# finsberg/fenicsx-beat

Measured on AMD Instinct MI355X. Metric: node_updates_per_sec, higher is better.
Workload: dtype f64

## Files before the change

fenicsx-beat_amd/csrc/beat_pde_rr.hip:

```cpp
#include "beat_pde_internal.h"

#include <algorithm>
#include <cmath>
#include <cstddef>
#include <cstdlib>

namespace {
using namespace beat_pde_detail;

constexpr int SEG = 62;

struct Coef {
  double c[15];
};

struct RGeom {
  int nx, ny, nz;
  int64_t plane;
  int ry;
  int nsegx, nrb, nchunks, zc;
  int total_waves, total_blocks;
  int z_lo_phys, z_hi_phys;
  int z_lo, z_hi;
  int part_off;
  int ghost_lo_tz, ghost_hi_tz;
  int nrg;
};

enum { RR_PDOT = 0, RR_RUPD = 1, RR_RHS = 2, RR_UDOT = 3, RR_PRUPD = 4 };

struct RArgs {
  const double* x;
  const double* x2;
  double* y;
  double* y2;
  const double* tab;
  const double* tab2;
  const double* dinv;
  Coef ci, ci2;
  double dinv_i;
  double cm, omt_dt, dt;
  const double* w[BEAT_MAX_STIM];
  double amp[BEAT_MAX_STIM];
  int nstim;
  double* partials;
  double* st;
  double* alphas;
  int slot;
  const double* e;
  const double* taba;
  Coef cia;
};

struct RKernArgs {
  RGeom g;
  RArgs a;
  const double* X;
  const double* X2;
  double* Y;
  double* Y2;
};

__device__ __forceinline__ double from_left(double v) {
  const int lo = __builtin_amdgcn_update_dpp(0, __double2loint(v), 0x138, 0xf, 0xf, true);
  const int hi = __builtin_amdgcn_update_dpp(0, __double2hiint(v), 0x138, 0xf, 0xf, true);
  return __hiloint2double(hi, lo);
}
__device__ __forceinline__ double from_right(double v) {
  const int lo = __builtin_amdgcn_update_dpp(0, __double2loint(v), 0x130, 0xf, 0xf, true);
  const int hi = __builtin_amdgcn_update_dpp(0, __double2hiint(v), 0x130, 0xf, 0xf, true);
  return __hiloint2double(hi, lo);
}

#ifndef BEAT_RR_BUF
#define BEAT_RR_BUF 2
#endif
typedef int rr_v2i __attribute__((ext_vector_type(2)));
[[maybe_unused]] constexpr unsigned RR_OOB = 0x80000000u;
#ifndef BEAT_RR_NT
#define BEAT_RR_NT 2
#endif
__device__ __forceinline__ void rr_store(double* p, double v) {
#if BEAT_RR_NT & 2
  __builtin_nontemporal_store(v, p);
#else
  *p = v;
#endif
}
__device__ __forceinline__ double rr_buf_load(const double* base, unsigned bytes, unsigned off) {
  const __amdgpu_buffer_rsrc_t r = __builtin_amdgcn_make_buffer_rsrc((void*)base, 0, (int)bytes, 0x00020000);
  const rr_v2i v = __builtin_amdgcn_raw_buffer_load_b64(r, (int)off, 0, (BEAT_RR_NT & 1) ? 2 : 0);
  return __hiloint2double(v.y, v.x);
}

#ifndef BEAT_RR_ALIGN
#define BEAT_RR_ALIGN 1
#endif
__device__ __forceinline__ double from_left_h(double v, double h, int src_lane) {
  const int lo = __builtin_amdgcn_update_dpp(__builtin_amdgcn_readlane(__double2loint(h), src_lane), __double2loint(v), 0x138, 0xf, 0xf, false);
  const int hi = __builtin_amdgcn_update_dpp(__builtin_amdgcn_readlane(__double2hiint(h), src_lane), __double2hiint(v), 0x138, 0xf, 0xf, false);
  return __hiloint2double(hi, lo);
}
__device__ __forceinline__ double from_right_h(double v, double h, int src_lane) {
  const int lo = __builtin_amdgcn_update_dpp(__builtin_amdgcn_readlane(__double2loint(h), src_lane), __double2loint(v), 0x130, 0xf, 0xf, false);
  const int hi = __builtin_amdgcn_update_dpp(__builtin_amdgcn_readlane(__double2hiint(h), src_lane), __double2hiint(v), 0x130, 0xf, 0xf, false);
  return __hiloint2double(hi, lo);
}
#ifndef BEAT_RR_ALIGN_RHS
#define BEAT_RR_ALIGN_RHS 0
#endif
constexpr bool rr_aligned_mode(int mode) {
  return BEAT_RR_ALIGN == 1 && BEAT_RR_BUF != 0 && (mode == 0 || mode == 1 || mode == 3 || mode == 4 || (mode == 2 && BEAT_RR_ALIGN_RHS == 1));
}

__device__ __forceinline__ int axis_type3(int i, int n, int lo_phys, int hi_phys) {
  if (n == 1 && lo_phys && hi_phys) return 1;
  if (i == 0 && lo_phys) return 0;
  if (i == n - 1 && hi_phys) return 2;
  return 1;
}

__device__ __forceinline__ int xcd_block(int b, int total) {
  const int per = (total + 7) >> 3;
  return (b & 7) * per + (b >> 3);
}

#ifndef BEAT_RR_WAVES_RHS
#define BEAT_RR_WAVES_RHS 3
#endif
#ifndef BEAT_RR_WAVES_IT
#define BEAT_RR_WAVES_IT 1
#endif
template <int MODE, int RY, int PD, bool GUESS = false, bool PRED = false>
__global__ __launch_bounds__(BEAT_BLOCK, (GUESS && RY == 2 && PD == 1) ? BEAT_RR_WAVES_RHS : ((MODE == RR_PDOT || MODE == RR_RUPD) && PD == 1 ? BEAT_RR_WAVES_IT : 1)) void rr_kernel(RGeom g, RArgs a, const double* __restrict__ X,
                                                        const double* __restrict__ X2, double* __restrict__ Y,
                                                        double* __restrict__ Y2) {
  constexpr int NR = RY + 2;
  constexpr int NE = GUESS ? NR : 1;
  constexpr bool FORM = MODE == RR_PDOT || MODE == RR_UDOT || MODE == RR_PRUPD;
  constexpr bool OLD = MODE == RR_PDOT || MODE == RR_PRUPD;
  constexpr bool RAW = MODE == RR_UDOT || MODE == RR_PRUPD;
  constexpr int NW = RAW ? RY : 1;
  constexpr bool BUF = BEAT_RR_BUF == 1 || (BEAT_RR_BUF == 2 && (MODE != RR_RHS || BEAT_RR_ALIGN_RHS == 1));
  constexpr bool ALIGNED = rr_aligned_mode(MODE);
  static_assert(!ALIGNED || BUF, "aligned segments come with the raw-buffer loads");
  constexpr int SEGW = ALIGNED ? 64 : SEG;
  static_assert(!GUESS || MODE == RR_RHS, "the initial guess enters the right-hand side only");
  static_assert(!PRED || MODE == RR_PDOT, "the predicted-stop sums come with PDOT only");
  __shared__ double red[4];
  __shared__ double s_dinv[32];
  __shared__ double s_tab[27 * TABW];
  __shared__ double s_tab2[MODE == RR_RHS ? 27 * TABW : 1];
  __shared__ double s_taba[GUESS ? 27 * TABW : 1];
  __shared__ double s_rc[PRED ? 4 * 2 * RY * 64 : 1];
  __shared__ double s_acc[PRED ? 4 * 2 * 64 : 1];
  if (MODE != RR_RHS) {
    if (a.st[STOP] != 0.0) return;
  }
  if (PRED) s_acc[(threadIdx.x >> 6) * 128 + (threadIdx.x & 63)] = s_acc[(threadIdx.x >> 6) * 128 + 64 + (threadIdx.x & 63)] = 0.0;
  for (int i = threadIdx.x; i < 27 * TABW; i += BEAT_BLOCK) {
    s_tab[i] = a.tab[i];
    if (MODE == RR_RHS) s_tab2[i] = a.tab2[i];
    if (GUESS) s_taba[i] = a.taba[i];
  }
  if (threadIdx.x < 27) s_dinv[threadIdx.x] = a.dinv[threadIdx.x];
  __syncthreads();
  const int lane = threadIdx.x & 63;
  const int blk = xcd_block(blockIdx.x, g.total_blocks);
  const int w = blk * 4 + (threadIdx.x >> 6);
  int seg = w % g.nsegx;
  int rb = (w / g.nsegx) % g.nrb;
  int chunk = w / (g.nsegx * g.nrb);
  bool wave_ok = blk < g.total_blocks && w < g.total_waves;
  if (g.nrg > 0) {
    seg = blk % g.nsegx;
    rb = ((blk / g.nsegx) % g.nrg) * 4 + (int)(threadIdx.x >> 6);
    chunk = blk / (g.nsegx * g.nrg);
    wave_ok = blk < g.total_blocks && rb < g.nrb;
  }
  const int gx = seg * SEGW + (ALIGNED ? 0 : -1) + lane;
  const int y0 = rb * RY - 1;
  const int zb = g.z_lo + chunk * g.zc;
  const int ze = wave_ok ? min(zb + g.zc, g.z_hi) : zb;
  const bool x_in = wave_ok && gx >= 0 && gx < g.nx;
  const bool x_out = x_in && (ALIGNED || (lane >= 1 && lane <= SEG));
  const int tx = axis_type3(gx, g.nx, 1, 1);
  bool row_in[NR];
  int txy[NR];
  int off[NR];
  const int cx = min(max(gx, 0), g.nx - 1);
#pragma unroll
  for (int r = 0; r < NR; ++r) {
    const int gy = y0 + r;
    row_in[r] = x_in && gy >= 0 && gy < g.ny;
    txy[r] = tx + 3 * axis_type3(gy, g.ny, 1, 1);
    off[r] = min(max(gy, 0), g.ny - 1) * g.nx + cx;
    if constexpr (BUF) off[r] = row_in[r] ? (int)((unsigned)(gy * g.nx + gx) * 8u) : (int)RR_OOB;
  }
  [[maybe_unused]] const unsigned pbytes = (unsigned)(g.plane * 8);
  [[maybe_unused]] unsigned hoff = RR_OOB;
  [[maybe_unused]] int htxy = 13 % 9;
  if constexpr (ALIGNED) {
    const int hr = lane < 8 ? lane : lane - 8;
    const int hx = lane < 8 ? seg * SEGW - 1 : seg * SEGW + SEGW;
    const int hy = y0 + hr;
    const bool hv = wave_ok && (lane < NR || (lane >= 8 && lane < 8 + NR)) && hx >= 0 && hx < g.nx && hy >= 0 && hy < g.ny;
    hoff = hv ? (unsigned)(hy * g.nx + hx) * 8u : RR_OOB;
    htxy = axis_type3(min(max(hx, 0), g.nx - 1), g.nx, 1, 1) + 3 * axis_type3(min(max(hy, 0), g.ny - 1), g.ny, 1, 1);
  }
  double beta = 0.0, alpha = 0.0;
  if (OLD) beta = a.st[BETA];
  if (MODE == RR_PRUPD) alpha = a.st[ALPHA];
  if (MODE == RR_RUPD) {
    alpha = a.st[RZ] / a.st[PQ];
    if (blockIdx.x == 0 && threadIdx.x == 0) a.alphas[a.slot] = alpha;
  }
  const bool have_old = beta != 0.0;

  double acc0 = 0.0, acc1 = 0.0, acc2 = 0.0;
  double Cm[NR], C0[NR], Cp[NR], ra[PD][NR], rb2[PD][NR];
  double rvn[PD][RY];
  [[maybe_unused]] double Hm = 0.0, H0 = 0.0, Hp = 0.0, rha[PD], rhb[PD];
  [[maybe_unused]] double HEm = 0.0, HE0 = 0.0, HEp = 0.0;
#pragma unroll
  for (int u = 0; u < PD; ++u) rha[u] = rhb[u] = 0.0;
  double Rw0[NW], Rwp[NW];
#pragma unroll
  for (int j = 0; j < NW; ++j) Rw0[j] = Rwp[j] = 0.0;
  double Em[NE], E0[NE], Ep[NE], re1[PD][NE];
#pragma unroll
  for (int r = 0; r < NE; ++r) {
    Em[r] = E0[r] = Ep[r] = 0.0;
#pragma unroll
    for (int u = 0; u < PD; ++u) re1[u][r] = 0.0;
  }
#pragma unroll
  for (int r = 0; r < NR; ++r) {
    Cm[r] = C0[r] = Cp[r] = 0.0;
#pragma unroll
    for (int u = 0; u < PD; ++u) ra[u][r] = rb2[u][r] = 0.0;
  }
#pragma unroll
  for (int u = 0; u < PD; ++u)
#pragma unroll
    for (int j = 0; j < RY; ++j) rvn[u][j] = 0.0;
  for (int zz = zb - 2 - PD; zz < ze; zz += PD) {
#pragma unroll
  for (int u = 0; u < PD; ++u) {
    const int z = zz + u;
    if (z < ze) {
    const int k = z + 1;
    if (k >= zb - 1 && k <= ze) {
      [[maybe_unused]] const bool zok = (k >= 0 || !g.z_lo_phys) && (k < g.nz || !g.z_hi_phys);
      const int tz9 = 9 * (k < 0 ? g.ghost_lo_tz : k >= g.nz ? g.ghost_hi_tz : axis_type3(k, g.nz, g.z_lo_phys, g.z_hi_phys));
      const bool own_plane = (k >= zb && k < ze) || (k == -1 && zb == 0 && !g.z_lo_phys) ||
                             (k == g.nz && ze == g.nz && !g.z_hi_phys);
#pragma unroll
      for (int r = 0; r < NR; ++r) {
        double c = ra[u][r];
        if (RAW && r >= 1 && r <= RY) Rwp[RAW ? r - 1 : 0] = c;
        if (FORM) {
          const int type = txy[r] + tz9;
          const double di = s_dinv[type];
          c = have_old ? fma(beta, rb2[u][r], di * ra[u][r]) : di * ra[u][r];
        }
        if constexpr (!BUF) c = (zok && row_in[r]) ? c : 0.0;
        Cp[r] = c;
        if (GUESS) {
          constexpr int q = GUESS ? 1 : 0;
          if constexpr (BUF)
            Ep[r * q] = c + re1[u][r * q];
          else
            Ep[r * q] = (zok && row_in[r]) ? c + re1[u][r * q] : 0.0;
        }
        if (OLD) {
          if (own_plane && r >= 1 && r <= RY && x_out && row_in[r])
            rr_store(&Y[(int64_t)k * g.plane + (int64_t)(y0 + r) * g.nx + gx], c);
        }
        if (PRED && r >= 1 && r <= RY) s_rc[((((threadIdx.x >> 6) * 2 + (k & 1)) * RY) + r - 1) * 64 + lane] = ra[u][r];
      }
      if constexpr (ALIGNED) {
        double hc = rha[u];
        if (FORM) {
          const double di = s_dinv[htxy + tz9];
          hc = have_old ? fma(beta, rhb[u], di * rha[u]) : di * rha[u];
        }
        Hp = hc;
        if (GUESS) HEp = hc + rhb[u];
      }
    }
    double rv[RY];
    if (MODE == RR_RUPD) {
#pragma unroll
      for (int j = 0; j < RY; ++j) rv[j] = rvn[u][j];
      if (z + PD >= zb && z + PD < ze) {
        const double* __restrict__ br = X2 + (int64_t)(z + PD) * g.plane;
#pragma unroll
        for (int j = 0; j < RY; ++j) rvn[u][j] = BUF ? rr_buf_load(br, pbytes, (unsigned)off[j + 1]) : br[off[j + 1]];
      }
    }
    {
      const int kf = k + PD;
      if (kf >= zb - 1 && kf <= ze) {
        const int cz = min(max(kf, -1), g.nz);
        const double* __restrict__ bx = X + (int64_t)cz * g.plane;
        const double* __restrict__ bx2 = (OLD && have_old) ? X2 + (int64_t)cz * g.plane : bx;
        if constexpr (BUF) {
          const unsigned pb = ((kf >= 0 || !g.z_lo_phys) && (kf < g.nz || !g.z_hi_phys)) ? pbytes : 0u;
#pragma unroll
          for (int r = 0; r < NR; ++r) {
            ra[u][r] = rr_buf_load(bx, pb, (unsigned)off[r]);
            if (OLD) rb2[u][r] = rr_buf_load(bx2, pb, (unsigned)off[r]);
          }
          if constexpr (ALIGNED) {
            rha[u] = rr_buf_load(bx, pb, hoff);
            if (OLD) rhb[u] = rr_buf_load(bx2, pb, hoff);
            if (GUESS) rhb[u] = rr_buf_load(X2 + (int64_t)cz * g.plane, pb, hoff);
          }
          if (GUESS) {
            const double* __restrict__ b1 = X2 + (int64_t)cz * g.plane;
#pragma unroll
            for (int r = 0; r < NR; ++r) re1[u][r < NE ? r : 0] = rr_buf_load(b1, pb, (unsigned)off[r]);
          }
        } else {
#pragma unroll
          for (int r = 0; r < NR; ++r) {
            ra[u][r] = bx[off[r]];
            if (OLD) rb2[u][r] = bx2[off[r]];
          }
          if (GUESS) {
            const double* __restrict__ b1 = X2 + (int64_t)cz * g.plane;
#pragma unroll
            for (int r = 0; r < NR; ++r) re1[u][r < NE ? r : 0] = b1[off[r]];
          }
        }
      }
    }
    if (z >= zb) {
    typedef const __attribute__((address_space(4))) char* KArgPtr;
    KArgPtr ka = (KArgPtr)__builtin_amdgcn_kernarg_segment_ptr();
    asm volatile("" : "+s"(ka));
    const RArgs& az = MODE == RR_RHS ? *(const RArgs*)(ka + offsetof(RKernArgs, a)) : a;
    double L0[NR], R0[NR], Rp[NR], Lm[NR];
#pragma unroll
    for (int r = 0; r < NR - 1; ++r) {
      L0[r] = ALIGNED ? from_left_h(C0[r], H0, r) : from_left(C0[r]);
      Lm[r] = ALIGNED ? from_left_h(Cm[r], Hm, r) : from_left(Cm[r]);
    }
#pragma unroll
    for (int r = 1; r < NR; ++r) {
      R0[r] = ALIGNED ? from_right_h(C0[r], H0, 8 + r) : from_right(C0[r]);
      Rp[r] = ALIGNED ? from_right_h(Cp[r], Hp, 8 + r) : from_right(Cp[r]);
    }
    double eL0[NE], eR0[NE], eRp[NE], eLm[NE];
    if (GUESS) {
#pragma unroll
      for (int r = 0; r < NE - 1; ++r) {
        eL0[r] = ALIGNED ? from_left_h(E0[r], HE0, r) : from_left(E0[r]);
        eLm[r] = ALIGNED ? from_left_h(Em[r], HEm, r) : from_left(Em[r]);
      }
#pragma unroll
      for (int r = 1; r < NE; ++r) {
        eR0[r] = ALIGNED ? from_right_h(E0[r], HE0, 8 + r) : from_right(E0[r]);
        eRp[r] = ALIGNED ? from_right_h(Ep[r], HEp, 8 + r) : from_right(Ep[r]);
      }
    }
    const int tz = axis_type3(z, g.nz, g.z_lo_phys, g.z_hi_phys);
#pragma unroll
    for (int j = 0; j < RY; ++j) {
      const int r = j + 1;
      double v[15];
      v[0] = C0[r];
      v[1] = R0[r];
      v[2] = L0[r];
      v[3] = C0[r + 1];
      v[4] = C0[r - 1];
      v[5] = Cp[r];
      v[6] = Cm[r];
      v[7] = R0[r + 1];
      v[8] = L0[r - 1];
      v[9] = Cp[r + 1];
      v[10] = Cm[r - 1];
      v[11] = Rp[r];
      v[12] = Lm[r];
      v[13] = Rp[r + 1];
      v[14] = Lm[r - 1];
      if (x_out && row_in[r]) {
        const int type = txy[r] + 9 * tz;
        const int64_t gi = (int64_t)z * g.plane + (int64_t)(y0 + r) * g.nx + gx;
        double s = 0.0;
#pragma unroll
        for (int k = 0; k < 15; ++k) s = fma(az.ci.c[k], v[k], s);
        if (MODE == RR_RHS) {
          double s2 = 0.0;
          if (!GUESS) {
#pragma unroll
            for (int k = 0; k < 15; ++k) s2 = fma(az.ci2.c[k], v[k], s2);
          }
          double di = s_dinv[13];
          if (type != 13) {
            s = 0.0;
            s2 = 0.0;
#pragma unroll
            for (int k = 0; k < 15; ++k) {
              s = fma(s_tab[type * TABW + k], v[k], s);
              if (!GUESS) s2 = fma(s_tab2[type * TABW + k], v[k], s2);
            }
            di = s_dinv[type];
          }
          double stim = 0.0;
          for (int k = 0; k < az.nstim; ++k) stim = fma(az.amp[k], az.w[k][gi], stim);
          const double b = GUESS ? fma(az.dt, stim, s) : az.cm * s - az.omt_dt * s2 + az.dt * stim;
          double rr = GUESS ? b : az.dt * (stim - s2);
          if (GUESS) {
            constexpr int q = GUESS ? 1 : 0;
            const int re_ = r * q, rp = (r + 1) * q, rm = (r - 1) * q;
            double ev[15];
            ev[0] = E0[re_];
            ev[1] = eR0[re_];
            ev[2] = eL0[re_];
            ev[3] = E0[rp];
            ev[4] = E0[rm];
            ev[5] = Ep[re_];
            ev[6] = Em[re_];
            ev[7] = eR0[rp];
            ev[8] = eL0[rm];
            ev[9] = Ep[rp];
            ev[10] = Em[rm];
            ev[11] = eRp[re_];
            ev[12] = eLm[re_];
            ev[13] = eRp[rp];
            ev[14] = eLm[rm];
            double se = 0.0;
            if (type != 13) {
#pragma unroll
              for (int k = 0; k < 15; ++k) se = fma(s_taba[type * TABW + k], ev[k], se);
            } else {
#pragma unroll
              for (int k = 0; k < 15; ++k) se = fma(az.cia.c[k], ev[k], se);
            }
            rr -= se;
          }
          const double zz = di * rr;
          rr_store(&Y[gi], rr);
          if (Y2 != nullptr) Y2[gi] = v[0];
          acc0 = fma(b, b, acc0);
          acc1 = fma(rr, zz, acc1);
          acc2 = fma(rr, rr, acc2);
        } else {
          double di = s_dinv[13];
          if (type != 13) {
            s = 0.0;
#pragma unroll
            for (int k = 0; k < 15; ++k) s = fma(s_tab[type * TABW + k], v[k], s);
            di = s_dinv[type];
          }
          if (MODE == RR_PDOT) {
            acc0 = fma(v[0], s, acc0);
            if (PRED) {
              double* sa = &s_acc[(threadIdx.x >> 6) * 128 + lane];
              sa[0] = fma(s_rc[((((threadIdx.x >> 6) * 2 + (z & 1)) * RY) + j) * 64 + lane], s, sa[0]);
              sa[64] = fma(s, s, sa[64]);
            }
          } else if (MODE == RR_UDOT) {
            const double ri = Rw0[RAW ? j : 0];
            acc0 = fma(v[0], s, acc0);
            acc1 = fma(ri, v[0], acc1);
            acc2 = fma(ri, ri, acc2);
          } else if (MODE == RR_PRUPD) {
            rr_store(&Y2[gi], fma(-alpha, s, Rw0[RAW ? j : 0]));
          } else {
            const double ri = fma(-alpha, s, rv[j]);
            rr_store(&Y[gi], ri);
            acc0 = fma(ri * di, ri, acc0);
            acc1 = fma(ri, ri, acc1);
          }
        }
      }
    }
    }
#pragma unroll
    for (int r = 0; r < NR; ++r) {
      Cm[r] = C0[r];
      C0[r] = Cp[r];
    }
    if constexpr (ALIGNED) {
      Hm = H0;
      H0 = Hp;
      if (GUESS) {
        HEm = HE0;
        HE0 = HEp;
      }
    }
    if (GUESS) {
#pragma unroll
      for (int r = 0; r < NE; ++r) {
        Em[r] = E0[r];
        E0[r] = Ep[r];
      }
    }
    if (RAW) {
#pragma unroll
      for (int j = 0; j < NW; ++j) Rw0[j] = Rwp[j];
    }
    }
  }
  }

  if (PRED) {
    acc1 = s_acc[(threadIdx.x >> 6) * 128 + (threadIdx.x & 63)];
    acc2 = s_acc[(threadIdx.x >> 6) * 128 + 64 + (threadIdx.x & 63)];
  }
  if (MODE == RR_PDOT && !PRED) {
    const double s0 = beat_block_sum(acc0, red);
    if (threadIdx.x == 0) a.partials[g.part_off + blockIdx.x] = s0;
  } else if (MODE == RR_RUPD) {
    const double s0 = beat_block_sum(acc0, red);
    const double s1 = beat_block_sum(acc1, red);
    if (threadIdx.x == 0) {
      a.partials[g.part_off + blockIdx.x] = s0;
      a.partials[BEAT_MAX_PARTIALS + g.part_off + blockIdx.x] = s1;
    }
  } else if (MODE == RR_PRUPD) {
  } else {
    const double s0 = beat_block_sum(acc0, red);
    const double s1 = beat_block_sum(acc1, red);
    const double s2 = beat_block_sum(acc2, red);
    if (threadIdx.x == 0) {
      a.partials[g.part_off + blockIdx.x] = s0;
      a.partials[BEAT_MAX_PARTIALS + g.part_off + blockIdx.x] = s1;
      a.partials[2 * BEAT_MAX_PARTIALS + g.part_off + blockIdx.x] = s2;
    }
  }
}

__global__ void rr_next_kernel(double* st) {
  if (st[STOP] != 0.0) return;
  st[BETA] = st[RZN] / st[RZ];
  st[RZ] = st[RZN];
  st[RR] = st[RRN];
  st[ITERS] += 1.0;
  const double tr = st[RTOL] * st[RTOL] * st[BB];
  if (st[RR] <= st[TOL2]) {
    st[STOP] = 1.0;
    st[REASON] = st[RR] <= tr ? 2.0 : 3.0;
  } else if (st[ITERS] >= st[MAXIT]) {
    st[STOP] = 1.0;
    st[REASON] = -3.0;
  }
}

__global__ void rr_merged_next_kernel(double* st, double* alphas, int slot) {
  if (st[STOP] != 0.0) return;
  const double g = st[RZN], d = st[PQ], rr = st[RRN];
  st[RR] = rr;
  const double tr = st[RTOL] * st[RTOL] * st[BB];
  if (rr <= st[TOL2]) {
    st[STOP] = 1.0;
    st[REASON] = rr <= tr ? 2.0 : 3.0;
    return;
  }
  if (st[ITERS] >= st[MAXIT]) {
    st[STOP] = 1.0;
    st[REASON] = -3.0;
    return;
  }
  const bool first = st[ITERS] == 0.0;
  const double beta = first ? 0.0 : g / st[RZ];
  const double alpha = first ? g / d : g / (d - beta * g / st[ALPHA]);
  st[BETA] = beta;
  st[ALPHA] = alpha;
  st[RZ] = g;
  alphas[slot] = alpha;
  st[NUPD] += 1.0;
  st[ITERS] += 1.0;
}

int rr_rows(int64_t nodes) {
  static const int forced = [] {
    const char* e = std::getenv("BEAT_RR_RY");
    const int v = e ? std::atoi(e) : 0;
    return (v == 2 || v == 4) ? v : 0;
  }();
  if (forced) return forced;
  return nodes >= ((int64_t)64 << 20) ? 4 : 2;
}

int rr_target_blocks(int64_t nodes) {
  if (const char* e = std::getenv("BEAT_RR_BLOCKS")) return std::max(1, std::atoi(e));
  return nodes >= ((int64_t)64 << 20) ? 4096 : 2048;
}

int rr_prefetch() {
  static const int pd = [] {
    const char* e = std::getenv("BEAT_RR_PD");
    const int v = e ? std::atoi(e) : 1;
    return (v >= 1 && v <= 3) ? v : 1;
  }();
  return pd;
}

int rr_by_rows_mask() {
  static const int mask = [] {
    const char* e = std::getenv("BEAT_RR_BY_ROWS");
    return e ? std::atoi(e) : 0;
  }();
  return mask;
}

RGeom make_geom(const beat_pde* pde, int z_lo, int z_hi, int part_off, int rows = 0, int mode = -1) {
  const Geom& f = pde->g;
  RGeom g{};
  const int64_t nodes = (int64_t)f.nx * f.ny * f.nz;
  const int RY = g.ry = rows ? rows : rr_rows(nodes);
  g.nx = f.nx;
  g.ny = f.ny;
  g.nz = f.nz;
  g.plane = f.plane;
  g.z_lo_phys = f.z_lo_phys;
  g.z_hi_phys = f.z_hi_phys;
  g.z_lo = z_lo;
  g.z_hi = z_hi;
  g.part_off = part_off;
  g.ghost_lo_tz = pde->ghost_lo_tz;
  g.ghost_hi_tz = pde->ghost_hi_tz;
  const int segw = (mode >= 0 && rr_aligned_mode(mode)) ? 64 : SEG;
  g.nsegx = (f.nx + segw - 1) / segw;
  g.nrb = (f.ny + RY - 1) / RY;
  const int nzr = std::max(0, z_hi - z_lo);
  g.nrg = (mode >= 0 && ((rr_by_rows_mask() >> mode) & 1)) ? (g.nrb + 3) / 4 : 0;
  const int64_t per_layer = g.nrg > 0 ? (int64_t)g.nsegx * g.nrg : ((int64_t)g.nsegx * g.nrb + 3) / 4;
  const int target = rr_target_blocks(nodes);
  int nchunks = (int)std::max<int64_t>(1, (target + per_layer - 1) / per_layer);
  nchunks = std::max(1, std::min(nchunks, nzr));
  g.zc = std::max(1, (nzr + nchunks - 1) / nchunks);
  g.nchunks = (nzr + g.zc - 1) / g.zc;
  while ((int64_t)g.nsegx * g.nrb * g.nchunks > (int64_t)2 * BEAT_MAX_PARTIALS && g.nchunks > 1) {
    g.zc *= 2;
    g.nchunks = (nzr + g.zc - 1) / g.zc;
  }
  g.total_waves = g.nsegx * g.nrb * g.nchunks;
  g.total_blocks = (g.total_waves + 3) / 4;
  if (g.nrg > 0) {
    g.total_blocks = g.nsegx * g.nrg * g.nchunks;
    g.total_waves = g.total_blocks * 4;
  }
  return g;
}

RGeom make_geom(const beat_pde* pde) { return make_geom(pde, 0, pde->g.nz, 0); }

inline int grid_blocks(const RGeom& g) { return ((g.total_blocks + 7) / 8) * 8; }
inline int blocks_written(const RGeom& g) { return g.total_blocks > 0 ? grid_blocks(g) : 0; }

Coef interior_row(const double* tab) {
  Coef c;
  for (int k = 0; k < 15; ++k) c.c[k] = tab[13 * 15 + k];
  return c;
}

RArgs rr_operator_args(const beat_pde* pde, double* dev_st) {
  RArgs a{};
  a.tab = pde->d_tab(0);
  a.dinv = pde->d_dinv();
  a.ci = interior_row(pde->h_A);
  a.dinv_i = pde->h_dinv[13];
  a.partials = pde->ctx->d_partials;
  a.st = dev_st;
  return a;
}

template <int MODE, bool GUESS = false, bool PRED = false>
void launch_rr(const beat_pde* pde, const RGeom& g, const RArgs& a) {
  if (g.total_blocks <= 0) return;
  const dim3 grid((unsigned)grid_blocks(g)), block(BEAT_BLOCK);
  hipStream_t s = pde->ctx->stream;
#define BEAT_RR_LAUNCH(RYV, PDV) \
  BEAT_KERNEL((rr_kernel<MODE, RYV, PDV, GUESS, PRED>), grid, block, 0, s, g, a, a.x, GUESS ? a.e : a.x2, a.y, a.y2)
  const int pd = rr_prefetch();
  if (g.ry == 2) {
    if (pd == 2) BEAT_RR_LAUNCH(2, 2); else if (pd == 3) BEAT_RR_LAUNCH(2, 3); else BEAT_RR_LAUNCH(2, 1);
  } else {
    if (pd == 2) BEAT_RR_LAUNCH(4, 2); else if (pd == 3) BEAT_RR_LAUNCH(4, 3); else BEAT_RR_LAUNCH(4, 1);
  }
#undef BEAT_RR_LAUNCH
}
}

bool beat_rr_available(const beat_pde* pde) {
  if (pde->var || pde->pc_ncoef != 1) return false;
  if (const char* e = std::getenv("BEAT_RR")) {
    if (e[0] == '0') return false;
  }
  const RGeom g = make_geom(pde);
  const RGeom gb = make_geom(pde, 0, 1, 0);
  return (int64_t)grid_blocks(g) + 2 * grid_blocks(gb) <= BEAT_MAX_PARTIALS;
}

int beat_rr_rhs(beat_pde* pde, const double* dev_v_prev, const double* const* host_dev_stim_w, const double* host_stim_amp,
                int n_stim, double* dev_x, double* dev_r, double* dev_st, int part, const PcgStart* start) {
  BEAT_REQUIRE(start == nullptr || part < 0, "only a right-hand side in one part starts the solve");
  const GuessTerms& gt = pde->guess;
  const bool guess = gt.d != nullptr && gt.use_e;
  static const int guess_rows = [] {
    const char* e = std::getenv("BEAT_RR_GUESS_RY");
    const int v = e ? std::atoi(e) : 2;
    return v == 4 ? 4 : 2;
  }();
  const int rows = guess ? guess_rows : 0;
  RArgs a{};
  a.x = dev_v_prev;
  a.y = dev_r;
  a.y2 = (dev_x == dev_v_prev) ? nullptr : dev_x;
  a.tab = pde->d_tab(2);
  a.tab2 = pde->d_tab(3);
  a.dinv = pde->d_dinv();
  a.ci = interior_row(pde->h_mass);
  a.ci2 = interior_row(pde->h_stiff);
  a.dinv_i = pde->h_dinv[13];
  a.cm = pde->C_m;
  a.omt_dt = (1.0 - pde->theta) * pde->dt;
  a.dt = pde->dt;
  beat_fill_stimuli(a, host_dev_stim_w, host_stim_amp, n_stim);
  a.partials = pde->ctx->d_partials;
  a.st = dev_st;
  if (guess) {
    a.tab = pde->d_tab(1);
    a.ci = interior_row(pde->h_B);
    a.e = gt.e;
    a.taba = pde->d_tab(0);
    a.cia = interior_row(pde->h_A);
  }
  auto launch = [&](int z_lo, int z_hi, int part_off) {
    const RGeom g = make_geom(pde, z_lo, z_hi, part_off, rows, RR_RHS);
    if (guess)
      launch_rr<RR_RHS, true>(pde, g, a);
    else
      launch_rr<RR_RHS>(pde, g, a);
    return blocks_written(g);
  };
  int count = 0;
  if (int rc = beat_launch_parts(pde, PASS_RR_RHS, part, launch, &count)) return rc;
  return part == 0 ? BEAT_OK : beat_pde_launch_reduce(pde, count, 3, dev_st, nullptr, ScalarStep::begin(dev_st, start));
}

double beat_rr_predict_bound(const beat_pde* pde) {
  const Geom& f = pde->g;
  int depth = 0;
  auto chain = [&](const RGeom& g) {
    const int per_thread = (grid_blocks(g) + BEAT_BLOCK - 1) / BEAT_BLOCK;
    depth = std::max(depth, g.zc * g.ry + 8 + per_thread + 8);
  };
  chain(make_geom(pde, 0, f.nz, 0, 0, RR_RHS));
  chain(make_geom(pde, 0, f.nz, 0, 2, RR_RHS));
  chain(make_geom(pde, 0, f.nz, 0, 4, RR_RHS));
  chain(make_geom(pde, 0, f.nz, 0, 0, RR_PDOT));
  chain(make_geom(pde, 0, f.nz, 0, 0, RR_RUPD));
  return 4.0 * (2.0 * depth + 8.0) * std::ldexp(1.0, -53);
}

int beat_rr_pdot_part(beat_pde* pde, double* dev_st, const double* dev_r, const double* dev_p_old, double* dev_p_new,
                      int part, int slot) {
  const Geom& f = pde->g;
  const bool pred = slot >= 0 && pde->predict_stop && f.z_lo_phys && f.z_hi_phys;
  if (pred && pde->predict_c <= 0.0) pde->predict_c = beat_rr_predict_bound(pde);
  RArgs a = rr_operator_args(pde, dev_st);
  a.x = dev_r;
  a.x2 = dev_p_old;
  a.y = dev_p_new;
  auto launch = [&](int z_lo, int z_hi, int part_off) {
    const RGeom g = make_geom(pde, z_lo, z_hi, part_off, 0, RR_PDOT);
    if (pred)
      launch_rr<RR_PDOT, false, true>(pde, g, a);
    else
      launch_rr<RR_PDOT>(pde, g, a);
    return blocks_written(g);
  };
  int count = 0;
  if (int rc = beat_launch_parts(pde, PASS_RR_PDOT, part, launch, &count)) return rc;
  if (part == 0) return BEAT_OK;
  if (pred) {
    static_assert(RQ == PQS + 1 && QQ == PQS + 2, "the three sums are reduced into one run of slots");
    ScalarStep predict{ScalarStep::PREDICT, dev_st};
    predict.alpha_slot = pde->d_alphas + slot;
    predict.bound_c = pde->predict_c;
    return beat_pde_launch_reduce(pde, count, 3, dev_st + PQS, dev_st, predict);
  }
  return beat_pde_launch_reduce(pde, count, 1, dev_st + PQ, dev_st);
}

int beat_rr_pdot(beat_pde* pde, double* dev_st, const double* dev_r, const double* dev_p_old, double* dev_p_new, int slot) {
  if (int rc = beat_rr_pdot_part(pde, dev_st, dev_r, dev_p_old, dev_p_new, 0, slot)) return rc;
  return beat_rr_pdot_part(pde, dev_st, dev_r, dev_p_old, dev_p_new, 1, slot);
}

int beat_rr_rupd(beat_pde* pde, double* dev_st, const double* dev_r, double* dev_r_new, const double* dev_p, int slot,
                 bool roll) {
  const RGeom g = make_geom(pde, 0, pde->g.nz, 0, 0, RR_RUPD);
  RArgs a = rr_operator_args(pde, dev_st);
  a.x = dev_p;
  a.x2 = dev_r;
  a.y = dev_r_new;
  a.alphas = pde->d_alphas;
  a.slot = slot;
  launch_rr<RR_RUPD>(pde, g, a);
  BEAT_LAUNCH_CHECK();
  return beat_pde_launch_reduce(pde, grid_blocks(g), 2, dev_st + RZN, dev_st, ScalarStep::after_update(dev_st, roll));
}

int beat_rr_udot_part(beat_pde* pde, double* dev_st, const double* dev_r, int part) {
  static_assert(RZN == PQ + 1 && RRN == PQ + 2, "the three sums travel as one all-reduce of dev_st[PQ..RRN]");
  RArgs a = rr_operator_args(pde, dev_st);
  a.x = dev_r;
  a.x2 = dev_r;
  auto launch = [&](int z_lo, int z_hi, int part_off) {
    const RGeom g = make_geom(pde, z_lo, z_hi, part_off, 0, RR_UDOT);
    launch_rr<RR_UDOT>(pde, g, a);
    return blocks_written(g);
  };
  int count = 0;
  if (int rc = beat_launch_parts(pde, PASS_RR_UDOT, part, launch, &count)) return rc;
  return part == 0 ? BEAT_OK : beat_pde_launch_reduce(pde, count, 3, dev_st + PQ, dev_st);
}

int beat_rr_merged_next(beat_pde* pde, double* dev_st, int slot) {
  BEAT_KERNEL(rr_merged_next_kernel, dim3(1), dim3(1), 0, pde->ctx->stream, dev_st, pde->d_alphas, slot);
  BEAT_LAUNCH_CHECK();
  return BEAT_OK;
}

int beat_rr_prupd(beat_pde* pde, double* dev_st, const double* dev_r, const double* dev_p_old, double* dev_p_new,
                  double* dev_r_new) {
  const RGeom g = make_geom(pde, 0, pde->g.nz, 0, 0, RR_PRUPD);
  RArgs a = rr_operator_args(pde, dev_st);
  a.x = dev_r;
  a.x2 = dev_p_old;
  a.y = dev_p_new;
  a.y2 = dev_r_new;
  launch_rr<RR_PRUPD>(pde, g, a);
  BEAT_LAUNCH_CHECK();
  return BEAT_OK;
}

int beat_rr_next(beat_pde* pde, double* dev_st) {
  BEAT_KERNEL(rr_next_kernel, dim3(1), dim3(1), 0, pde->ctx->stream, dev_st);
  BEAT_LAUNCH_CHECK();
  return BEAT_OK;
}
```

Measured before the change: 11.61 billion.

## Replace readlane halo exchange with DPP row shifts and trim per-thread address math

The halo lanes are remapped so each row's halo value sits within the same 16-lane DPP row, which lets the per-row readlane broadcasts be replaced by row_shl/row_shr DPP moves. Per-row flat offsets drop the x component, which is now added as a separate vector byte offset on top of a uniform base, so the scalar unit handles the row addressing. The wave index goes through readfirstlane and row validity is recomputed from a scalar y0. An optional register-rotation path, off by default, avoids the plane-shift copies. The point is to cut VALU and readlane work and VGPR pressure, at the cost of more complex and fragile lane bookkeeping.

```diff
diff --git a/fenicsx-beat_amd/csrc/beat_pde_rr.hip b/fenicsx-beat_amd/csrc/beat_pde_rr.hip
--- a/fenicsx-beat_amd/csrc/beat_pde_rr.hip
+++ b/fenicsx-beat_amd/csrc/beat_pde_rr.hip
@@ -4,6 +4,7 @@
 #include <cmath>
 #include <cstddef>
 #include <cstdlib>
+#include <type_traits>
 
 namespace {
 using namespace beat_pde_detail;
@@ -96,15 +97,41 @@
 #ifndef BEAT_RR_ALIGN
 #define BEAT_RR_ALIGN 1
 #endif
-__device__ __forceinline__ double from_left_h(double v, double h, int src_lane) {
-  const int lo = __builtin_amdgcn_update_dpp(__builtin_amdgcn_readlane(__double2loint(h), src_lane), __double2loint(v), 0x138, 0xf, 0xf, false);
-  const int hi = __builtin_amdgcn_update_dpp(__builtin_amdgcn_readlane(__double2hiint(h), src_lane), __double2hiint(v), 0x138, 0xf, 0xf, false);
+__device__ __forceinline__ int rr_row_shl(int h, int r) {
+  switch (r) {
+    case 1: return __builtin_amdgcn_update_dpp(0, h, 0x101, 0xf, 0xf, true);
+    case 2: return __builtin_amdgcn_update_dpp(0, h, 0x102, 0xf, 0xf, true);
+    case 3: return __builtin_amdgcn_update_dpp(0, h, 0x103, 0xf, 0xf, true);
+    case 4: return __builtin_amdgcn_update_dpp(0, h, 0x104, 0xf, 0xf, true);
+    case 5: return __builtin_amdgcn_update_dpp(0, h, 0x105, 0xf, 0xf, true);
+    default: return h;
+  }
+}
+__device__ __forceinline__ int rr_row_shr(int h, int r) {
+  switch (r) {
+    case 1: return __builtin_amdgcn_update_dpp(0, h, 0x111, 0xf, 0xf, true);
+    case 2: return __builtin_amdgcn_update_dpp(0, h, 0x112, 0xf, 0xf, true);
+    case 3: return __builtin_amdgcn_update_dpp(0, h, 0x113, 0xf, 0xf, true);
+    case 4: return __builtin_amdgcn_update_dpp(0, h, 0x114, 0xf, 0xf, true);
+    case 5: return __builtin_amdgcn_update_dpp(0, h, 0x115, 0xf, 0xf, true);
+    default: return h;
+  }
+}
+__device__ __forceinline__ double from_left_h(double v, double h, int r) {
+  const int lo = __builtin_amdgcn_update_dpp(rr_row_shl(__double2loint(h), r), __double2loint(v), 0x138, 0xf, 0xf, false);
+  const int hi = __builtin_amdgcn_update_dpp(rr_row_shl(__double2hiint(h), r), __double2hiint(v), 0x138, 0xf, 0xf, false);
   return __hiloint2double(hi, lo);
 }
-__device__ __forceinline__ double from_right_h(double v, double h, int src_lane) {
-  const int lo = __builtin_amdgcn_update_dpp(__builtin_amdgcn_readlane(__double2loint(h), src_lane), __double2loint(v), 0x130, 0xf, 0xf, false);
-  const int hi = __builtin_amdgcn_update_dpp(__builtin_amdgcn_readlane(__double2hiint(h), src_lane), __double2hiint(v), 0x130, 0xf, 0xf, false);
+__device__ __forceinline__ double from_right_h(double v, double h, int r) {
+  const int lo = __builtin_amdgcn_update_dpp(rr_row_shr(__double2loint(h), r), __double2loint(v), 0x130, 0xf, 0xf, false);
+  const int hi = __builtin_amdgcn_update_dpp(rr_row_shr(__double2hiint(h), r), __double2hiint(v), 0x130, 0xf, 0xf, false);
   return __hiloint2double(hi, lo);
+}
+template <class T>
+__device__ __forceinline__ T* rr_at(T* uniform_base, unsigned& byte_off) {
+  typedef typename std::conditional<std::is_const<T>::value, const char, char>::type Byte;
+  asm volatile("" : "+v"(byte_off));
+  return (T*)((Byte*)uniform_base + byte_off);
 }
 #ifndef BEAT_RR_ALIGN_RHS
 #define BEAT_RR_ALIGN_RHS 0
@@ -125,6 +152,9 @@
   return (b & 7) * per + (b >> 3);
 }
 
+#ifndef BEAT_RR_ROTATE
+#define BEAT_RR_ROTATE 0
+#endif
 #ifndef BEAT_RR_WAVES_RHS
 #define BEAT_RR_WAVES_RHS 3
 #endif
@@ -157,7 +187,9 @@
   if (MODE != RR_RHS) {
     if (a.st[STOP] != 0.0) return;
   }
-  if (PRED) s_acc[(threadIdx.x >> 6) * 128 + (threadIdx.x & 63)] = s_acc[(threadIdx.x >> 6) * 128 + 64 + (threadIdx.x & 63)] = 0.0;
+  const int lane = threadIdx.x & 63;
+  const int wv = __builtin_amdgcn_readfirstlane((int)(threadIdx.x >> 6));
+  if (PRED) s_acc[wv * 128 + lane] = s_acc[wv * 128 + 64 + lane] = 0.0;
   for (int i = threadIdx.x; i < 27 * TABW; i += BEAT_BLOCK) {
     s_tab[i] = a.tab[i];
     if (MODE == RR_RHS) s_tab2[i] = a.tab2[i];
@@ -165,16 +197,15 @@
   }
   if (threadIdx.x < 27) s_dinv[threadIdx.x] = a.dinv[threadIdx.x];
   __syncthreads();
-  const int lane = threadIdx.x & 63;
   const int blk = xcd_block(blockIdx.x, g.total_blocks);
-  const int w = blk * 4 + (threadIdx.x >> 6);
+  const int w = blk * 4 + wv;
   int seg = w % g.nsegx;
   int rb = (w / g.nsegx) % g.nrb;
   int chunk = w / (g.nsegx * g.nrb);
   bool wave_ok = blk < g.total_blocks && w < g.total_waves;
   if (g.nrg > 0) {
     seg = blk % g.nsegx;
-    rb = ((blk / g.nsegx) % g.nrg) * 4 + (int)(threadIdx.x >> 6);
+    rb = ((blk / g.nsegx) % g.nrg) * 4 + wv;
     chunk = blk / (g.nsegx * g.nrg);
     wave_ok = blk < g.total_blocks && rb < g.nrb;
   }
@@ -189,22 +220,23 @@
   int txy[NR];
   int off[NR];
   const int cx = min(max(gx, 0), g.nx - 1);
+  [[maybe_unused]] unsigned gxb = (unsigned)gx * 8u, cxb = (unsigned)cx * 8u;
 #pragma unroll
   for (int r = 0; r < NR; ++r) {
     const int gy = y0 + r;
     row_in[r] = x_in && gy >= 0 && gy < g.ny;
     txy[r] = tx + 3 * axis_type3(gy, g.ny, 1, 1);
-    off[r] = min(max(gy, 0), g.ny - 1) * g.nx + cx;
+    off[r] = min(max(gy, 0), g.ny - 1) * g.nx;
     if constexpr (BUF) off[r] = row_in[r] ? (int)((unsigned)(gy * g.nx + gx) * 8u) : (int)RR_OOB;
   }
   [[maybe_unused]] const unsigned pbytes = (unsigned)(g.plane * 8);
   [[maybe_unused]] unsigned hoff = RR_OOB;
   [[maybe_unused]] int htxy = 13 % 9;
   if constexpr (ALIGNED) {
-    const int hr = lane < 8 ? lane : lane - 8;
-    const int hx = lane < 8 ? seg * SEGW - 1 : seg * SEGW + SEGW;
+    const int hr = lane < 32 ? lane : 63 - lane;
+    const int hx = lane < 32 ? seg * SEGW - 1 : seg * SEGW + SEGW;
     const int hy = y0 + hr;
-    const bool hv = wave_ok && (lane < NR || (lane >= 8 && lane < 8 + NR)) && hx >= 0 && hx < g.nx && hy >= 0 && hy < g.ny;
+    const bool hv = wave_ok && hr < NR && hx >= 0 && hx < g.nx && hy >= 0 && hy < g.ny;
     hoff = hv ? (unsigned)(hy * g.nx + hx) * 8u : RR_OOB;
     htxy = axis_type3(min(max(hx, 0), g.nx - 1), g.nx, 1, 1) + 3 * axis_type3(min(max(hy, 0), g.ny - 1), g.ny, 1, 1);
   }
@@ -218,25 +250,26 @@
   const bool have_old = beta != 0.0;
 
   double acc0 = 0.0, acc1 = 0.0, acc2 = 0.0;
-  double Cm[NR], C0[NR], Cp[NR], ra[PD][NR], rb2[PD][NR];
+  constexpr int ROT = (BEAT_RR_ROTATE == 1 && PD == 1) ? 3 : 1;
+  double CW[3][NR], ra[PD][NR], rb2[PD][NR];
   double rvn[PD][RY];
-  [[maybe_unused]] double Hm = 0.0, H0 = 0.0, Hp = 0.0, rha[PD], rhb[PD];
-  [[maybe_unused]] double HEm = 0.0, HE0 = 0.0, HEp = 0.0;
+  [[maybe_unused]] double HW[3] = {0.0, 0.0, 0.0}, rha[PD], rhb[PD];
+  [[maybe_unused]] double HEW[3] = {0.0, 0.0, 0.0};
 #pragma unroll
   for (int u = 0; u < PD; ++u) rha[u] = rhb[u] = 0.0;
-  double Rw0[NW], Rwp[NW];
-#pragma unroll
-  for (int j = 0; j < NW; ++j) Rw0[j] = Rwp[j] = 0.0;
-  double Em[NE], E0[NE], Ep[NE], re1[PD][NE];
+  double RW[3][NW];
+#pragma unroll
+  for (int j = 0; j < NW; ++j) RW[0][j] = RW[1][j] = RW[2][j] = 0.0;
+  double EW[3][NE], re1[PD][NE];
 #pragma unroll
   for (int r = 0; r < NE; ++r) {
-    Em[r] = E0[r] = Ep[r] = 0.0;
+    EW[0][r] = EW[1][r] = EW[2][r] = 0.0;
 #pragma unroll
     for (int u = 0; u < PD; ++u) re1[u][r] = 0.0;
   }
 #pragma unroll
   for (int r = 0; r < NR; ++r) {
-    Cm[r] = C0[r] = Cp[r] = 0.0;
+    CW[0][r] = CW[1][r] = CW[2][r] = 0.0;
 #pragma unroll
     for (int u = 0; u < PD; ++u) ra[u][r] = rb2[u][r] = 0.0;
   }
@@ -244,11 +277,21 @@
   for (int u = 0; u < PD; ++u)
 #pragma unroll
     for (int j = 0; j < RY; ++j) rvn[u][j] = 0.0;
-  for (int zz = zb - 2 - PD; zz < ze; zz += PD) {
+  for (int zz = zb - 2 - PD; zz < ze; zz += PD * ROT) {
+#pragma unroll
+  for (int ph = 0; ph < ROT; ++ph) {
 #pragma unroll
   for (int u = 0; u < PD; ++u) {
-    const int z = zz + u;
+    const int z = zz + ph * PD + u;
     if (z < ze) {
+    double(&Cm)[NR] = CW[ph % 3], (&C0)[NR] = CW[(ph + 1) % 3], (&Cp)[NR] = CW[(ph + 2) % 3];
+    double(&Em)[NE] = EW[ph % 3], (&E0)[NE] = EW[(ph + 1) % 3], (&Ep)[NE] = EW[(ph + 2) % 3];
+    double(&Rw0)[NW] = RW[(ph + 1) % 3], (&Rwp)[NW] = RW[(ph + 2) % 3];
+    [[maybe_unused]] double &Hm = HW[ph % 3], &H0 = HW[(ph + 1) % 3], &Hp = HW[(ph + 2) % 3];
+    [[maybe_unused]] double &HEm = HEW[ph % 3], &HE0 = HEW[(ph + 1) % 3], &HEp = HEW[(ph + 2) % 3];
+    int y0s = y0;
+    asm volatile("" : "+s"(y0s));
+    auto row_ok = [&](int r) { return (unsigned)(y0s + r) < (unsigned)g.ny; };
     const int k = z + 1;
     if (k >= zb - 1 && k <= ze) {
       [[maybe_unused]] const bool zok = (k >= 0 || !g.z_lo_phys) && (k < g.nz || !g.z_hi_phys);
@@ -264,20 +307,20 @@
           const double di = s_dinv[type];
           c = have_old ? fma(beta, rb2[u][r], di * ra[u][r]) : di * ra[u][r];
         }
-        if constexpr (!BUF) c = (zok && row_in[r]) ? c : 0.0;
+        if constexpr (!BUF) c = (zok && x_in && row_ok(r)) ? c : 0.0;
         Cp[r] = c;
         if (GUESS) {
           constexpr int q = GUESS ? 1 : 0;
           if constexpr (BUF)
             Ep[r * q] = c + re1[u][r * q];
           else
-            Ep[r * q] = (zok && row_in[r]) ? c + re1[u][r * q] : 0.0;
+            Ep[r * q] = (zok && x_in && row_ok(r)) ? c + re1[u][r * q] : 0.0;
         }
         if (OLD) {
-          if (own_plane && r >= 1 && r <= RY && x_out && row_in[r])
-            rr_store(&Y[(int64_t)k * g.plane + (int64_t)(y0 + r) * g.nx + gx], c);
+          if (own_plane && r >= 1 && r <= RY && row_ok(r) && x_out)
+            rr_store(rr_at(Y + ((int64_t)k * g.plane + (int64_t)(y0s + r) * g.nx), gxb), c);
         }
-        if (PRED && r >= 1 && r <= RY) s_rc[((((threadIdx.x >> 6) * 2 + (k & 1)) * RY) + r - 1) * 64 + lane] = ra[u][r];
+        if (PRED && r >= 1 && r <= RY) s_rc[(((wv * 2 + (k & 1)) * RY) + r - 1) * 64 + lane] = ra[u][r];
       }
       if constexpr (ALIGNED) {
         double hc = rha[u];
@@ -296,7 +339,7 @@
       if (z + PD >= zb && z + PD < ze) {
         const double* __restrict__ br = X2 + (int64_t)(z + PD) * g.plane;
 #pragma unroll
-        for (int j = 0; j < RY; ++j) rvn[u][j] = BUF ? rr_buf_load(br, pbytes, (unsigned)off[j + 1]) : br[off[j + 1]];
+        for (int j = 0; j < RY; ++j) rvn[u][j] = BUF ? rr_buf_load(br, pbytes, (unsigned)off[j + 1]) : *rr_at(br + off[j + 1], cxb);
       }
     }
     {
@@ -325,13 +368,13 @@
         } else {
 #pragma unroll
           for (int r = 0; r < NR; ++r) {
-            ra[u][r] = bx[off[r]];
-            if (OLD) rb2[u][r] = bx2[off[r]];
+            ra[u][r] = *rr_at(bx + off[r], cxb);
+            if (OLD) rb2[u][r] = *rr_at(bx2 + off[r], cxb);
           }
           if (GUESS) {
             const double* __restrict__ b1 = X2 + (int64_t)cz * g.plane;
 #pragma unroll
-            for (int r = 0; r < NR; ++r) re1[u][r < NE ? r : 0] = b1[off[r]];
+            for (int r = 0; r < NR; ++r) re1[u][r < NE ? r : 0] = *rr_at(b1 + off[r], cxb);
           }
         }
       }
@@ -349,8 +392,8 @@
     }
 #pragma unroll
     for (int r = 1; r < NR; ++r) {
-      R0[r] = ALIGNED ? from_right_h(C0[r], H0, 8 + r) : from_right(C0[r]);
-      Rp[r] = ALIGNED ? from_right_h(Cp[r], Hp, 8 + r) : from_right(Cp[r]);
+      R0[r] = ALIGNED ? from_right_h(C0[r], H0, r) : from_right(C0[r]);
+      Rp[r] = ALIGNED ? from_right_h(Cp[r], Hp, r) : from_right(Cp[r]);
     }
     double eL0[NE], eR0[NE], eRp[NE], eLm[NE];
     if (GUESS) {
@@ -361,8 +404,8 @@
       }
 #pragma unroll
       for (int r = 1; r < NE; ++r) {
-        eR0[r] = ALIGNED ? from_right_h(E0[r], HE0, 8 + r) : from_right(E0[r]);
-        eRp[r] = ALIGNED ? from_right_h(Ep[r], HEp, 8 + r) : from_right(Ep[r]);
+        eR0[r] = ALIGNED ? from_right_h(E0[r], HE0, r) : from_right(E0[r]);
+        eRp[r] = ALIGNED ? from_right_h(Ep[r], HEp, r) : from_right(Ep[r]);
       }
     }
     const int tz = axis_type3(z, g.nz, g.z_lo_phys, g.z_hi_phys);
@@ -385,9 +428,9 @@
       v[12] = Lm[r];
       v[13] = Rp[r + 1];
       v[14] = Lm[r - 1];
-      if (x_out && row_in[r]) {
+      if (row_ok(r) && x_out) {
         const int type = txy[r] + 9 * tz;
-        const int64_t gi = (int64_t)z * g.plane + (int64_t)(y0 + r) * g.nx + gx;
+        const int64_t gi = (int64_t)z * g.plane + (int64_t)(y0s + r) * g.nx;
         double s = 0.0;
 #pragma unroll
         for (int k = 0; k < 15; ++k) s = fma(az.ci.c[k], v[k], s);
@@ -409,7 +452,7 @@
             di = s_dinv[type];
           }
           double stim = 0.0;
-          for (int k = 0; k < az.nstim; ++k) stim = fma(az.amp[k], az.w[k][gi], stim);
+          for (int k = 0; k < az.nstim; ++k) stim = fma(az.amp[k], *rr_at(az.w[k] + gi, gxb), stim);
           const double b = GUESS ? fma(az.dt, stim, s) : az.cm * s - az.omt_dt * s2 + az.dt * stim;
           double rr = GUESS ? b : az.dt * (stim - s2);
           if (GUESS) {
@@ -442,8 +485,8 @@
             rr -= se;
           }
           const double zz = di * rr;
-          rr_store(&Y[gi], rr);
-          if (Y2 != nullptr) Y2[gi] = v[0];
+          rr_store(rr_at(Y + gi, gxb), rr);
+          if (Y2 != nullptr) *rr_at(Y2 + gi, gxb) = v[0];
           acc0 = fma(b, b, acc0);
           acc1 = fma(rr, zz, acc1);
           acc2 = fma(rr, rr, acc2);
@@ -458,8 +501,8 @@
           if (MODE == RR_PDOT) {
             acc0 = fma(v[0], s, acc0);
             if (PRED) {
-              double* sa = &s_acc[(threadIdx.x >> 6) * 128 + lane];
-              sa[0] = fma(s_rc[((((threadIdx.x >> 6) * 2 + (z & 1)) * RY) + j) * 64 + lane], s, sa[0]);
+              double* sa = &s_acc[wv * 128 + lane];
+              sa[0] = fma(s_rc[(((wv * 2 + (z & 1)) * RY) + j) * 64 + lane], s, sa[0]);
               sa[64] = fma(s, s, sa[64]);
             }
           } else if (MODE == RR_UDOT) {
@@ -468,10 +511,10 @@
             acc1 = fma(ri, v[0], acc1);
             acc2 = fma(ri, ri, acc2);
           } else if (MODE == RR_PRUPD) {
-            rr_store(&Y2[gi], fma(-alpha, s, Rw0[RAW ? j : 0]));
+            rr_store(rr_at(Y2 + gi, gxb), fma(-alpha, s, Rw0[RAW ? j : 0]));
           } else {
             const double ri = fma(-alpha, s, rv[j]);
-            rr_store(&Y[gi], ri);
+            rr_store(rr_at(Y + gi, gxb), ri);
             acc0 = fma(ri * di, ri, acc0);
             acc1 = fma(ri, ri, acc1);
           }
@@ -479,37 +522,40 @@
       }
     }
     }
-#pragma unroll
-    for (int r = 0; r < NR; ++r) {
-      Cm[r] = C0[r];
-      C0[r] = Cp[r];
-    }
-    if constexpr (ALIGNED) {
-      Hm = H0;
-      H0 = Hp;
+    if constexpr (ROT == 1) {
+#pragma unroll
+      for (int r = 0; r < NR; ++r) {
+        Cm[r] = C0[r];
+        C0[r] = Cp[r];
+      }
+      if constexpr (ALIGNED) {
+        Hm = H0;
+        H0 = Hp;
+        if (GUESS) {
+          HEm = HE0;
+          HE0 = HEp;
+        }
+      }
       if (GUESS) {
-        HEm = HE0;
-        HE0 = HEp;
-      }
-    }
-    if (GUESS) {
-#pragma unroll
-      for (int r = 0; r < NE; ++r) {
-        Em[r] = E0[r];
-        E0[r] = Ep[r];
-      }
-    }
-    if (RAW) {
-#pragma unroll
-      for (int j = 0; j < NW; ++j) Rw0[j] = Rwp[j];
-    }
-    }
+#pragma unroll
+        for (int r = 0; r < NE; ++r) {
+          Em[r] = E0[r];
+          E0[r] = Ep[r];
+        }
+      }
+      if (RAW) {
+#pragma unroll
+        for (int j = 0; j < NW; ++j) Rw0[j] = Rwp[j];
+      }
+    }
+    }
+  }
   }
   }
 
   if (PRED) {
-    acc1 = s_acc[(threadIdx.x >> 6) * 128 + (threadIdx.x & 63)];
-    acc2 = s_acc[(threadIdx.x >> 6) * 128 + 64 + (threadIdx.x & 63)];
+    acc1 = s_acc[wv * 128 + lane];
+    acc2 = s_acc[wv * 128 + 64 + lane];
   }
   if (MODE == RR_PDOT && !PRED) {
     const double s0 = beat_block_sum(acc0, red);
```

New measurement: 11.53 billion. No clear change (-0.6%).
